# IntelLabs/bayesian-torch

Measured on AMD Instinct MI355X. Metric: MC-samples/sec (Bayesian-ResNet18, 224^2, bs=64), higher is better.
Workload: dtype bf16

## Files before the change

bayesian_torch_amd/_lib.py:

```python
import ctypes
import os

_HERE = os.path.dirname(os.path.abspath(__file__))
_LIB = None

KIND_REPARAM, KIND_FLIPOUT = 0, 1
ACT_F32, ACT_BF16 = 0, 1
PREC_F32, PREC_BF16, PREC_BF16X3 = 0, 1, 2
PREC_CODE = {"f32": 0, "bf16": 1, "bf16x3": 2}
FLAG_TRANSPOSED, FLAG_KL_ACCUM, FLAG_ROWFUSE, FLAG_OUT_F32, FLAG_OUT_BF16, FLAG_GATHER, FLAG_SWAP_SIGNS, FLAG_CONCURRENT = 1, 2, 4, 8, 16, 32, 64, 128
FLAG_REVERSE = 256
E_UNSUPPORTED = -3
STREAM_EPS_W, STREAM_EPS_B, STREAM_SIGN_IN, STREAM_SIGN_OUT = 0, 1, 2, 3
ABI_VERSION = 9
FLAG_LANES_SHIFT = 16
FLAG_LANES_MASK = 0xff << FLAG_LANES_SHIFT
SAMPLE_SKIP_MU = 1


class BtxError(RuntimeError):
    pass


class Geom(ctypes.Structure):
# ... 76 lines not shown


class OptimItem(ctypes.Structure):
    _fields_ = [("p", ctypes.c_void_p), ("g", ctypes.c_void_p), ("state0", ctypes.c_void_p), ("state1", ctypes.c_void_p),
                ("n", ctypes.c_int64)]


class BucketItem(ctypes.Structure):
    _fields_ = [("src", ctypes.c_void_p), ("offset", ctypes.c_int64), ("n", ctypes.c_int64)]


class OptimHyper(ctypes.Structure):
    _fields_ = [(n, ctypes.c_float) for n in ("neg_lr", "wd", "decay_mul", "one_m_b1", "b2", "one_m_b2", "eps", "neg_step_size",
                                              "bc2s", "momentum", "one_m_damp")] + \
               [("flags", ctypes.c_uint32), ("reserved", ctypes.c_uint32 * 4)]


OPT_MAXIMIZE, OPT_NESTEROV, OPT_DECOUPLED, OPT_FIRST_STEP, OPT_COUPLED_WD = 1, 2, 4, 8, 16
OPTIM_CHUNK, OPTIM_MAX_ITEMS = 4096, 65536
Q8_BIAS_NONE, Q8_BIAS_MU, Q8_BIAS_SIGMA_EPS = 0, 1, 2

EXPORTS = ("btx_abi_version", "btx_strerror", "btx_kl_workspace_bytes", "btx_kl_gauss", "btx_kl_model_workspace_bytes",
           "btx_kl_gauss_model", "btx_kl_gauss_model_bwd", "btx_contract_wgrad",
           "btx_contract_workspace_bytes", "btx_contract_fwd", "btx_contract_fwd_ex", "btx_contract_fwd_lanes", "btx_contract_pool_shape", "btx_contract_plan_info", "btx_out_shape", "btx_fill_eps", "btx_fill_sign", "btx_rho_grad",
           "btx_mc_packed_floats", "btx_mc_accumulate", "btx_mc_accumulate_lanes", "btx_sampled_w_bytes", "btx_sample_weights", "btx_sampled_w_bytes_lanes", "btx_sample_weights_lanes", "btx_rowfuse_pack", "btx_maxpool2d_cl", "btx_avgpool_global_cl",
           "btx_bn_workspace_bytes", "btx_bn_train_fwd", "btx_bn_train_bwd", "btx_dgrad_weights",
           "btx_wgrad_workspace_bytes", "btx_contract_wgrad_ws", "btx_maxpool2d_cl_train", "btx_maxpool2d_cl_bwd",
           "btx_lstm_workspace_bytes", "btx_lstm_fwd", "btx_lstm_train_saved_bytes", "btx_lstm_train_workspace_bytes",
           "btx_lstm_fwd_train", "btx_lstm_bwd",
           "btx_calib_workspace_bytes", "btx_avu_fwd", "btx_avu_bwd", "btx_eau_fwd", "btx_eau_bwd",
           "btx_q8_weight_row_bytes", "btx_q8_quantize_act", "btx_q8_sample_weights", "btx_q8_contract",
           "btx_q8_add", "btx_q8_contract_res", "btx_q8_maxpool2d_cl", "btx_q8_avgpool2d_cl",
           "btx_q8_sample_delta", "btx_q8_contract_flipout",
           "btx_optim_sgd", "btx_optim_adam", "btx_optim_grad_norm_workspace_bytes", "btx_optim_grad_norm",
           "btx_mcloss_workspace_bytes", "btx_mc_ce_fwd", "btx_mc_ce_bwd", "btx_avu_mc_fwd", "btx_avu_mc_bwd",
           "btx_bias_grad_workspace_bytes", "btx_bias_grad",
           "btx_bucket_pack", "btx_bucket_unpack")


def lib_path():
    return os.environ.get("BTX_LIB") or os.path.join(_HERE, "libbtx.so")


def lib():
    global _LIB
    if _LIB is not None:
        return _LIB
# ... 16 lines not shown
    L.btx_kl_gauss_model.restype = i32
    L.btx_kl_gauss_model.argtypes = [ctypes.POINTER(KlItem), i32, vp, vp, sz, vp]
    L.btx_kl_gauss_model_bwd.restype = i32
    L.btx_kl_gauss_model_bwd.argtypes = [ctypes.POINTER(KlItem), i32, vp, vp]
    L.btx_contract_wgrad.restype = i32
    L.btx_contract_wgrad.argtypes = [i32, ctypes.POINTER(Geom), vp, vp, vp, vp, vp, vp, ctypes.POINTER(Rng),
                                     ctypes.POINTER(Noise), i32, u32, vp]
    L.btx_contract_wgrad_ws.restype = i32
    L.btx_contract_wgrad_ws.argtypes = [i32, ctypes.POINTER(Geom), vp, vp, vp, vp, vp, vp, ctypes.POINTER(Rng),
                                        ctypes.POINTER(Noise), i32, u32, vp, sz, vp, vp, vp]
    L.btx_wgrad_workspace_bytes.restype = sz
    L.btx_wgrad_workspace_bytes.argtypes = [i32, ctypes.POINTER(Geom), i32, u32]
    L.btx_contract_workspace_bytes.restype = sz
    L.btx_contract_workspace_bytes.argtypes = [ctypes.POINTER(Geom), i32, i32, i32, u32]
    L.btx_contract_fwd.restype = i32
    L.btx_contract_fwd.argtypes = [i32, ctypes.POINTER(Geom), vp, vp, vp, vp, vp, vp, ctypes.POINTER(Rng),
                                   ctypes.POINTER(Noise), i32, i32, u32, vp, sz, vp]
    L.btx_contract_fwd_ex.restype = i32
    L.btx_contract_fwd_ex.argtypes = L.btx_contract_fwd.argtypes + [ctypes.POINTER(Epilogue)]
    L.btx_contract_fwd_lanes.restype = i32
    L.btx_contract_fwd_lanes.argtypes = L.btx_contract_fwd_ex.argtypes + [ctypes.POINTER(Lanes)]
    L.btx_contract_plan_info.restype = i32
    L.btx_contract_plan_info.argtypes = [i32, ctypes.POINTER(Geom), i32, i32, u32, ctypes.POINTER(Epilogue), ctypes.POINTER(PlanInfo)]
    L.btx_contract_pool_shape.restype = i32
    L.btx_contract_pool_shape.argtypes = [ctypes.POINTER(Geom), i32, i32, u32] + [ctypes.POINTER(ctypes.c_int32)] * 2
    L.btx_out_shape.restype = i32
    L.btx_out_shape.argtypes = [ctypes.POINTER(Geom), u32] + [ctypes.POINTER(ctypes.c_int32)] * 3
    L.btx_fill_eps.restype = i32
    L.btx_fill_eps.argtypes = [vp, sz, ctypes.POINTER(Rng), u32, vp]
    L.btx_rho_grad.restype = i32
    L.btx_rho_grad.argtypes = [vp, vp, vp, sz, ctypes.POINTER(Rng), u32, vp]
    L.btx_fill_sign.restype = i32
    L.btx_fill_sign.argtypes = [vp, sz, ctypes.POINTER(Rng), u32, vp]
    L.btx_mc_packed_floats.restype = sz
    L.btx_mc_packed_floats.argtypes = [i32, i32]
    L.btx_sampled_w_bytes.restype = sz
    L.btx_sampled_w_bytes.argtypes = [ctypes.POINTER(Geom), i32, i32]
    L.btx_sample_weights.restype = i32
    L.btx_sample_weights.argtypes = [ctypes.POINTER(SampleItem), i32, ctypes.POINTER(Rng), i32, vp]
    L.btx_sampled_w_bytes_lanes.restype = sz
    L.btx_sampled_w_bytes_lanes.argtypes = [ctypes.POINTER(Geom), i32, i32, i32]
    L.btx_sample_weights_lanes.restype = i32
    L.btx_sample_weights_lanes.argtypes = [ctypes.POINTER(SampleItem), i32, ctypes.POINTER(Rng), i32, vp, i32, u32]
    L.btx_rowfuse_pack.restype = i32
    L.btx_rowfuse_pack.argtypes = [vp, i32, ctypes.POINTER(ctypes.c_int64), i32, i32, i32, i32, vp, i32, i32, i32, i32, i32,
                                   i32, vp]
# ... 106 lines not shown
```

bayesian_torch_amd/csrc/btx_api.hip:

```cpp
#include <hip/hip_runtime.h>
#include <math.h>
#include <string.h>
#include "../../include/btx.h"
#include <stdlib.h>
#include "btx_contract.h"
#include "btx_rng.h"
#include "btx_presample.h"

using namespace btx;

static int contract_fwd_impl(int kind, const BtxGeom* g, const void* x, const float* mu_w, const float* rho_w,
                             const float* mu_b, const float* rho_b, void* out, const BtxRng* rng, const BtxNoise* noise,
                             int act_dtype, int prec, uint32_t flags, void* ws, size_t ws_bytes, void* stream,
                             const BtxEpilogue* ep, const BtxLanes* ln) {
  if (!g || !x || !mu_w || !rho_w || !out || !rng) return BTX_E_NULL;
  const int lanes = ln ? ln->n : 1;
  if ((mu_b == nullptr) != (rho_b == nullptr)) return BTX_E_NULL;
  const uintptr_t al = (uintptr_t)x | (uintptr_t)mu_w | (uintptr_t)rho_w | (uintptr_t)out |
                       (uintptr_t)(noise && noise->eps_w ? noise->eps_w : nullptr) |
                       (uintptr_t)(ep && ep->residual ? ep->residual : nullptr);
  FwdSel sel;
  int rc = select_fwd(kind, g, act_dtype, prec, flags, (al & 15) != 0, noise, ep, &sel);
  if (rc) return rc;
  const Plan& pl = sel.pl;
// ... 85 lines not shown
    case BTX_FAMILY_STEM: {
      const StemPlan& stp = sel.stp;
      p.pt_R = stp.R; p.pt_Rp = stp.Rp; p.pt_rtiles = stp.rtiles; p.pt_nw = stp.nw; p.pt_astage = stp.astage;
      p.st_sbytes = stp.sbytes; p.pt_lds = stp.lds; p.pt_PP = stp.patch_bytes;
      p.fd_rtiles = make_fastdiv((uint32_t)stp.rtiles);
      rc = launch(launch_contract_stem_f32, launch_contract_stem_bf16, launch_contract_stem_x3);
      break;
    }
    case BTX_FAMILY_PATCH:
    case BTX_FAMILY_TAPS:
    case BTX_FAMILY_TAPS2: {
      const PatchPlan& pt = sel.pt;
      p.pt_G = pt.G; p.pt_R = pt.R; p.pt_Rp = pt.Rp; p.pt_Wp = pt.Wp; p.pt_PP = pt.PP; p.pt_NI = pt.NI;
      p.fd_ptWp = make_fastdiv((uint32_t)pt.Wp); p.fd_ptRp = make_fastdiv((uint32_t)pt.Rp); p.fd_ptR = make_fastdiv((uint32_t)pt.R);
      p.fd_rtiles = make_fastdiv((uint32_t)pt.rtiles);
      p.pt_rtiles = pt.rtiles; p.pt_nw = pt.nw; p.pt_astage = pt.astage; p.pt_lds = pt.lds;
      p.pt_taps = pt.taps; p.pt_kg = pt.kg; p.pt_lds_g = pt.lds_g;
      p.pt_wide = (pt.taps == 33 || pt.taps == 332) ? pt.wide : 0;
      if (p.pt_wide) {
        p.fd_ntiles = make_fastdiv((uint32_t)(pl.ntiles / 2));
        p.fd_inner = make_fastdiv((uint32_t)((pl.ntiles / 2) * g->groups * pl.ksplits));
      }
      p.pt_tall = pt.tall; p.pt_P = pt.P; p.pt_Wt = pt.Wt; p.pt_ncs = pt.ncs;
      p.fd_P = make_fastdiv((uint32_t)pt.P); p.fd_Wt = make_fastdiv((uint32_t)pt.Wt); p.fd_ncs = make_fastdiv((uint32_t)pt.ncs);
      rc = launch(launch_contract_patch_f32, launch_contract_patch_bf16, launch_contract_patch_x3);
      break;
    }
    case BTX_FAMILY_GEMM8:
      p.pt_rtiles = sel.g8_pairs;
      p.fd_rtiles = make_fastdiv((uint32_t)sel.g8_pairs); p.fd_inner = make_fastdiv((uint32_t)(sel.g8_pairs * g->groups));
      rc = launch(launch_contract_gemm8_f32, launch_contract_gemm8_bf16, launch_contract_gemm8_x3);
      break;
    case BTX_FAMILY_DMA:
      rc = launch(launch_contract_dma_f32, launch_contract_dma_bf16, launch_contract_dma_x3);
      break;
    default: {
      const bool gen2 = sel.family == BTX_FAMILY_GATHER || (noise && (noise->eps_w || noise->sign_in));
      rc = (prec == BTX_PREC_BF16) ? launch_contract_bf16(kind, act_dtype == BTX_ACT_BF16, gen2, p, pl.nwg * lanes, st)
                                   : launch_contract_f32(kind, act_dtype == BTX_ACT_BF16, gen2, p, pl.nwg * lanes, st);
    }
  }
  if (rc) return rc;
  if (pl.ksplits > 1) {
    const long long total = (long long)pl.M * g->N;
    long long blocks = (total / 4 + 255) / 256;
    if (blocks > 2048) blocks = 2048;
// ... 122 lines not shown
```

bayesian_torch_amd/csrc/btx_contract.h:

```cpp
#pragma once
#include <hip/hip_runtime.h>
#include <stdint.h>
#include "btx_rng.h"
#include "btx_plan.h"

typedef __attribute__((ext_vector_type(8))) __bf16 bf16x8;
typedef __attribute__((ext_vector_type(4))) __bf16 bf16x4;
typedef __attribute__((ext_vector_type(4))) float f32x4;
typedef __attribute__((ext_vector_type(8))) float f32x8;
typedef __attribute__((ext_vector_type(16))) float f32x16;
typedef __attribute__((ext_vector_type(4))) uint32_t u32x4;
typedef __attribute__((ext_vector_type(2))) uint32_t u32x2;

namespace btx {

constexpr int NTHREADS = 512;
constexpr int ACTS_OFF = 0;
constexpr int SIGN_OFF = NG * BM * 16;
constexpr int WMU_OFF = SIGN_OFF + NG * BM * 4;
constexpr int WDL_OFF = WMU_OFF + NG * BN * 16;
constexpr int STAGE_BYTES = WDL_OFF + NG * BN * 16;
constexpr int LDS_BYTES = 2 * STAGE_BYTES;

struct FastDiv {
// ... 51 lines not shown
  int ep_relu;
  int out_bf16;
  int sign_unaligned;
  uint32_t x_bytes, w_bytes;
  int pt_G, pt_R, pt_Rp, pt_Wp, pt_PP, pt_NI, pt_rtiles;
  FastDiv fd_Wo, fd_Ho, fd_Do, fd_ptWp, fd_ptRp, fd_ptR;
  FastDiv fd_inner, fd_ksplits, fd_ntiles, fd_Cg, fd_KW, fd_KH, fd_rtiles;
  FastDiv fd_mtiles;
  int swap_signs;
  int par_major, par_Mq, par_Mqp, par_Hh, par_Wh;
  FastDiv fd_par_Mqp, fd_par_Hh, fd_par_Wh;
  FastDiv fd_sd, fd_sh, fd_sw;
  int wg_order;
  int pt_nw, pt_astage, pt_lds;
  int pt_kg;
  int pt_lds_g;
  int pt_taps;
  int pt_wide;
  int sp_Hq, sp_Wq;
  int st_sbytes;
  void* wt;
  uint32_t wt_bytes, wt_delta_off;
  int wt_ready;
  int pt_tall, pt_P, pt_Wt, pt_ncs;
  FastDiv fd_P, fd_Wt, fd_ncs;
  int lanes, lane_nwg;
  FastDiv fd_lane_nwg;
  long long lane_x, lane_out, lane_res, lane_wt, lane_partial;
  int lane_wt_delta;
  int reverse;
};

__device__ __forceinline__ uint32_t sample_word_scalar(const uint32_t* ptr) {
  return *(const __attribute__((address_space(4))) uint32_t*)(uintptr_t)ptr;
}

__device__ __forceinline__ int xcd_logical() {
  const int nwg = gridDim.x, L = blockIdx.x;
  const int q = nwg >> 3, r = nwg & 7, xcd = L & 7, slot = L >> 3;
  return (xcd < r ? xcd * (q + 1) : r * (q + 1) + (xcd - r) * q) + slot;
}

__device__ __forceinline__ ContractParams lane_view(const ContractParams& q, int& logical) {
  ContractParams p = q;
  if (q.reverse) logical = (int)gridDim.x - 1 - logical;
  if (q.lanes > 1) {
    uint32_t lane, loc;
// ... 687 lines not shown
```

bayesian_torch_amd/csrc/btx_contract_taps.h:

```cpp
#pragma once
#include <type_traits>
#include "btx_contract.h"
#include "btx_contract_dma.h"
#include "btx_epilogue.h"
#include "btx_mma.h"

namespace btx {

__device__ __forceinline__ void dma16s(__amdgpu_buffer_rsrc_t rsrc, uint32_t voff, uint32_t soff,
                                       unsigned char* lds_wave_base) {
  __builtin_amdgcn_raw_ptr_buffer_load_lds(rsrc, (__attribute__((address_space(3))) void*)lds_wave_base, 16, voff, soff,
                                           0, 0);
}

template <int N>
__device__ __forceinline__ void end_stage() {
  asm volatile("s_waitcnt vmcnt(%0)\n\ts_waitcnt lgkmcnt(0)\n\ts_barrier" ::"n"(N) : "memory");
}

template <int I, int N, class F>
__device__ __forceinline__ void static_for(F&& f) {
  if constexpr (I < N) {
    f(std::integral_constant<int, I>{});
    static_for<I + 1, N>(f);
// ... 30 lines not shown
  constexpr int ESZ = (int)sizeof(ACT);
  extern __shared__ __attribute__((aligned(16))) unsigned char smem_all[];

  uint32_t smp = p.sample;
  if (p.sample_ptr) smp = sample_word_scalar(p.sample_ptr);

  const int tid = threadIdx.x & 255;
  const int lane = tid & 63;
  const int l31 = lane & 31;
  const int h = lane >> 5;
  const int wave_all = __builtin_amdgcn_readfirstlane((int)(threadIdx.x >> 6));
  const int wave = wave_all & 3;
  const int kg = (KG == 1) ? 0 : (wave_all >> 2);
  unsigned char* const smem = smem_all + kg * p.pt_lds_g;

  uint32_t u_mtile, u_rem, u_split, u_ntile, u_group, u_t;
  const uint32_t ntg = (uint32_t)(WIDE ? p.ntiles >> 1 : p.ntiles);
  if (p.wg_order) fdivmod((uint32_t)logical, p.fd_mtiles, (uint32_t)p.mtiles, u_rem, u_mtile);
  else fdivmod((uint32_t)logical, p.fd_inner, ntg * (uint32_t)(p.groups * p.ksplits), u_mtile, u_rem);
  fdivmod(u_rem, p.fd_ksplits, (uint32_t)p.ksplits, u_t, u_split);
  fdivmod(u_t, p.fd_ntiles, ntg, u_group, u_ntile);
  const int mtile = (int)u_mtile, split = (int)u_split, ntile = (int)u_ntile, group = (int)u_group;

  const bool tall = p.pt_tall != 0;
  uint32_t u_ig, u_rt;
  if (tall) fdivmod((uint32_t)mtile, p.fd_ncs, (uint32_t)p.pt_ncs, u_rt, u_ig);
  else fdivmod((uint32_t)mtile, p.fd_rtiles, (uint32_t)p.pt_rtiles, u_ig, u_rt);
  const int img0 = tall ? 0 : (int)u_ig * p.pt_G, row0 = (int)u_rt * p.pt_R, col0 = tall ? (int)u_ig * p.pt_Wt : 0;
  auto patch_src = [&](int q, bool& ok) __attribute__((always_inline)) -> uint32_t {
    uint32_t ut, upc, ugi, upr;
    fdivmod((uint32_t)q, p.fd_ptWp, (uint32_t)p.pt_Wp, ut, upc);
    int img, ih, iw;
    if (tall) {
      fdivmod((uint32_t)row0 + ut, p.fd_P, (uint32_t)p.pt_P, ugi, upr);
      img = (int)ugi; ih = (int)upr - p.ph; iw = col0 + (int)upc - p.pw;
      ok = (int)ut < p.pt_Rp;
    } else {
      fdivmod(ut, p.fd_ptRp, (uint32_t)p.pt_Rp, ugi, upr);
      img = img0 + (int)ugi; ih = row0 + (int)upr - p.ph; iw = (int)upc - p.pw;
      ok = true;
    }
    ok = ok && img < p.NB && (unsigned)ih < (unsigned)p.H && (unsigned)iw < (unsigned)p.W;
    return (uint32_t)((img * p.H + ih) * p.W + iw);
  };
  const int ncb_total = p.Cg / BK;
  const int cb_per = p.kper / BK;
  const int cb0 = split * cb_per + kg * (cb_per / KG);
  const int ncb = (KG == 1) ? min(ncb_total, cb0 + cb_per) - cb0 : cb_per / KG;
  const int a_stage = p.pt_astage, s_stage = p.pt_astage >> 4;
  const int PT_A_OFF = 0, PT_S_OFF = 2 * a_stage, PT_W_OFF = 2 * a_stage + 2 * s_stage;
  const int PT_X_OFF = PT_W_OFF + PT_WD * DW_STAGE;

  const __amdgpu_buffer_rsrc_t x_rsrc = __builtin_amdgcn_make_buffer_rsrc((void*)p.x, 0, p.x_bytes, 0x00020000);
  const __amdgpu_buffer_rsrc_t wt_rsrc = __builtin_amdgcn_make_buffer_rsrc((void*)p.wt, 0, p.wt_bytes, 0x00020000);

  const uint32_t w_voff = (uint32_t)lane * 16u + (uint32_t)wave * 1024u;
  const uint32_t w_sbase = (uint32_t)(group * p.ntiles + (WIDE ? 2 * ntile : ntile)) * (uint32_t)(p.K / G) * 1024u;
// ... 69 lines not shown

  auto write_signs = [&](int slot, int cb) __attribute__((always_inline)) {
    if constexpr (KIND == 1) {
      unsigned char* ss = smem + PT_S_OFF + slot * s_stage;
#pragma unroll
      for (int j = 0; j < 2; ++j) {
        if (sg_ok[j]) {
          const uint32_t off = sg_off[j] + (uint32_t)(cb * BK);
          uint32_t w;
          if (p.sign_in) w = sign_word_explicit(p.sign_in, off, p.x_bytes / (uint32_t)ESZ);
          else w = btx_sign_word(off >> 5, rl.kin_a, rl.kin_b);
          if constexpr (G == 4) w <<= 8 * ((off >> 4) & 1);
          *(uint32_t*)(ss + (tid + NT * j) * 4) = w;
        }
      }
    }
  };

  int q0[MI];
#pragma unroll
  for (int mi = 0; mi < MI; ++mi) {
    const int pl = wave * 64 + mi * 32 + l31;
    uint32_t ut, uc, ugi, ur;
    if (tall) {
      fdivmod((uint32_t)pl, p.fd_Wt, (uint32_t)p.pt_Wt, ur, uc);
      q0[mi] = ((int)ur < p.pt_R) ? (int)ur * p.pt_Wp + (int)uc : 0;
    } else {
      fdivmod((uint32_t)pl, p.fd_Wo, (uint32_t)p.Wo, ut, uc);
      fdivmod(ut, p.fd_ptR, (uint32_t)p.pt_R, ugi, ur);
      const int c = (int)uc, r = (int)ur, gi = (int)ugi;
      const bool ok = (gi < p.pt_G) && (img0 + gi < p.NB) && (row0 + r < p.Ho);
      q0[mi] = ok ? (gi * p.pt_Rp + r) * p.pt_Wp + c : 0;
    }
  }
  const int row_step = p.dh * p.pt_Wp;

  constexpr bool ZI = (PREC == 1 && KG == 1);
  f32x16 accm[MI][2], accd[MI][2];
  auto clear_acc = [&](int a0) __attribute__((always_inline)) {
#pragma unroll
    for (int a = 0; a < MI; ++a)
#pragma unroll
      for (int b = 0; b < 2; ++b)
#pragma unroll
        for (int r = 0; r < 16; ++r)
          if (a >= a0) { accm[a][b][r] = 0.f; accd[a][b][r] = 0.f; }
  };
// ... 6 lines not shown
    const unsigned char* ss = smem + PT_S_OFF + aslot * s_stage;
    const unsigned char* ws = smem + PT_W_OFF + wsl * DW_STAGE;
    int q[MI];
#pragma unroll
    for (int mi = 0; mi < MI; ++mi) q[mi] = q0[mi] + toffv;
#pragma unroll
    for (int kk = 0; kk < NG / 2; ++kk) {
      const int row = 2 * kk + h;
#pragma unroll
      for (int mi = 0; mi < MIA; ++mi) f.a[kk][mi] = *(const u32x4*)(as + q[mi] * 64 + ((row ^ ((q[mi] >> 2) & 3)) * 16));
#pragma unroll
      for (int ni = 0; ni < 2; ++ni) f.wm[kk][ni] = *(const u32x4*)(ws + (row * BN + ni * 32 + l31) * 16);
    }
    if constexpr (KIND == 1) {
#pragma unroll
      for (int mi = 0; mi < MIA; ++mi) f.sw[mi] = *(const uint32_t*)(ss + q[mi] * 4);
    }
  };

  if (ncb > 0) {
    write_signs(0, cb0);
    asm volatile("s_waitcnt vmcnt(%0)\n\ts_waitcnt lgkmcnt(0)\n\ts_barrier" ::"n"(KG == 1 ? WOPS : 2 * WOPS) : "memory");
    Frag fa, fb;
    const int nvalid_px = tall ? p.pt_R * p.pt_Wt : min(p.pt_G, p.NB - img0) * min(p.pt_R, p.Ho - row0) * p.Wo;
    const bool mi1_dead = wave * 64 + 32 >= nvalid_px;
    auto kloop = [&](auto mia_tag) __attribute__((always_inline)) {
    constexpr int MIA = decltype(mia_tag)::value;
    if constexpr (KG == 1) load_frag(fa, 0, 0, 0, mia_tag);
    auto block = [&](auto par_tag, auto first_tag, int cbi, bool last) __attribute__((always_inline)) {
      constexpr int PAR = decltype(par_tag)::value;
      constexpr bool FIRST = decltype(first_tag)::value;
      static_for<0, T>([&](auto t_tag) __attribute__((always_inline)) {
        constexpr int t = decltype(t_tag)::value;
        constexpr int sp = (PAR * T + t) & 1;
        Frag& cur = (KG == 1 && sp) ? fb : fa;
        Frag& nxt = (KG == 1 && sp) ? fa : fb;
        asm volatile("" : "+v"(q0[0]), "+v"(q0[1]));
        constexpr int t3 = (t + 3) % T, c3 = (t + 3) / T;
        if constexpr (c3 == 0) {
          issue_w((uint32_t)t3, (uint32_t)(cb0 + cbi), (wslot + 3) & 3);
        } else {
          if (!last) issue_w((uint32_t)t3, (uint32_t)(cb0 + cbi + 1), (wslot + 3) & 3);
        }
        constexpr int KP = tp_pieces<T>(t);
        if constexpr (t < PST) {
          if (!last) {
            const uint32_t cboff = (uint32_t)((cb0 + cbi + 1) * BK * ESZ);
// ... 43 lines not shown
      block(P0{}, std::true_type{}, 0, ncb == 1);
      int cbi = 1;
      for (; cbi + 2 <= ncb; cbi += 2) {
        block(P1{}, std::false_type{}, cbi, false);
        block(P0{}, std::false_type{}, cbi + 1, cbi + 2 == ncb);
      }
      if (cbi < ncb) block(P1{}, std::false_type{}, cbi, true);
    } else {
      int cbi = 0;
      for (; cbi + 2 <= ncb; cbi += 2) {
        block(P0{}, std::false_type{}, cbi, false);
        block(P1{}, std::false_type{}, cbi + 1, cbi + 2 == ncb);
      }
      if (cbi < ncb) block(P0{}, std::false_type{}, cbi, true);
    }
    if (KG == 2 && kg == 0) asm volatile("s_barrier" ::: "memory");
    };
    if (mi1_dead) kloop(std::integral_constant<int, 1>{});
    else kloop(std::integral_constant<int, 2>{});
  }

  {
    BTX_SECTION_PARAMS(pe, logical2);
    const int nimg = min(pe.pt_G, pe.NB - img0), nrow = min(pe.pt_R, pe.Ho - row0);
    const int nvalid = nimg * nrow * pe.Wo;
    const uint32_t m0 = (uint32_t)(img0 * pe.Ho + row0) * (uint32_t)pe.Wo;
    const PixTall pmt = {pe, row0, col0};
    if constexpr (KG == 1) {
      if constexpr (WIDE) {
        float* const ba0 = (float*)(smem + NW * PT_EP_WAVE);
        float* const ba1 = ba0 + 4 * BN;
        {
          const bool has_bias = (split == 0) && (pe.mu_b != nullptr);
          const bool has_aff = (pe.ksplits == 1) && ((pe.ep_scale != nullptr) || (pe.ep_shift != nullptr));
          if (has_bias || has_aff) {
            if (tid < 64) ep_fill_constants<0>(pe, rl, ba0, tid, 2 * ntile, group, has_bias, has_aff);
            else if (tid < 128) ep_fill_constants<0>(pe, rl, ba1, tid - 64, 2 * ntile + 1, group, has_bias, has_aff);
          }
          __syncthreads();
        }
        if (tall) {
          staged_epilogue_pm<0, NW, PixTall>(pe, rl, accm, accm, smem, tid, wave, lane, 2 * ntile, group, split, pmt, -1, true, ba0);
          staged_epilogue_pm<0, NW, PixTall>(pe, rl, accd, accd, smem, tid, wave, lane, 2 * ntile + 1, group, split, pmt, -1, true, ba1);
        } else {
          staged_epilogue<0, NW>(pe, rl, accm, accm, smem, tid, wave, lane, 2 * ntile, group, split, m0, nvalid, -1, true, ba0);
          staged_epilogue<0, NW>(pe, rl, accd, accd, smem, tid, wave, lane, 2 * ntile + 1, group, split, m0, nvalid, -1, true, ba1);
        }
// ... 57 lines not shown
```

bayesian_torch_amd/csrc/btx_plan.cpp:

```cpp
#include <string.h>
#include "btx_plan.h"

namespace btx {

static inline long long plan_lanes(uint32_t flags) {
  const long long n = (flags >> BTX_FLAG_LANES_SHIFT) & 0xffu;
  return n > 1 ? n : 1;
}

static inline bool throughput_plan(uint32_t flags) { return (flags & BTX_FLAG_CONCURRENT) || plan_lanes(flags) > 1; }

static int split_k(long long base1, int units, int unit_cost, int max_split, bool full_splits, bool throughput, bool short_exit) {
  int ks = 1;
  long long best = -1;
  for (int c = 1; c <= max_split; ++c) {
    if (full_splits && units % c) continue;
    const int per = (units + c - 1) / c;
    const long long rounds = (base1 * c + SLOTS - 1) / SLOTS;
    const long long cost = rounds * (per * unit_cost + 4) + (c > 1 ? 1 : 0);
    if (best < 0 || cost < best) { best = cost; ks = c; }
    if (throughput && (base1 * c >= 64 || (short_exit && base1 * c >= 16 && per <= 16))) { ks = c; break; }
  }
  return ks;
}
// ... 40 lines not shown
static double tall_tile(const BtxGeom* g, const Plan& pl, int tp, int ppcap, PatchPlan* pt) {
  const int halo_r = (g->KH - 1) * g->dh, halo_c = (g->KW - 1) * g->dw;
  if (g->ph > halo_r) return 0.0;
  const int P = (g->H + g->ph > pl.Ho) ? g->H + g->ph : pl.Ho;
  const long long rows_total = (long long)(g->NB - 1) * P + pl.Ho;
  double best = 0.0;
  for (int ncs = 1; ncs <= 8; ++ncs) {
    const int Wt = (pl.Wo + ncs - 1) / ncs;
    if (Wt > tp || Wt < 4 || (ncs > 1 && Wt < 8)) continue;
    int R = tp / Wt;
    if (R > rows_total) R = (int)rows_total;
    while (R >= 1 && (R + halo_r) * (Wt + halo_c) > ppcap) --R;
    if (R < 1) continue;
    const long long rtiles = (rows_total + R - 1) / R;
    const double eff = (double)pl.M / ((double)rtiles * ncs * tp);
    if (eff > best * 1.01) {
      best = eff;
      pt->tall = 1; pt->P = P; pt->Wt = Wt; pt->ncs = ncs;
      pt->G = 1; pt->R = R; pt->Rp = R + halo_r; pt->Wp = Wt + halo_c; pt->PP = pt->Rp * pt->Wp;
      pt->rtiles = (int)rtiles;
    }
  }
  return best;
}
static bool patch_tile(const BtxGeom* g, const Plan& pl, int tp, int ppcap, PatchPlan* pt) {
  const int Ho = pl.Ho, Wo = pl.Wo;
  const int Wp = Wo + (g->KW - 1) * g->dw, halo_r = (g->KH - 1) * g->dh;
  if (Wo > tp || Wp * (1 + halo_r) > ppcap) return false;
  int G = 1, R;
  if (Ho * Wo <= tp / 2 || (Ho * Wo <= tp && (Ho + halo_r) * Wp <= ppcap)) {
    R = Ho;
    const int Rp = R + halo_r;
    if (Rp * Wp > ppcap) return false;
    G = tp / (Ho * Wo);
    if (G > ppcap / (Rp * Wp)) G = ppcap / (Rp * Wp);
    if (G > g->NB) G = g->NB;
    if (G < 1) return false;
  } else {
    int rmax = tp / Wo;
    const int rfit = ppcap / Wp - halo_r;
    if (rfit < rmax) rmax = rfit;
    if (rmax > Ho) rmax = Ho;
    if (rmax < 1) return false;
    const int nrt = (Ho + rmax - 1) / rmax;
    R = (Ho + nrt - 1) / nrt;
    auto mfma_tiles = [&](int r) {
// ... 44 lines not shown
}
static bool patch_split_k(const BtxGeom* g, int prec, uint32_t flags, int T, Plan* pl, const PatchPlan& pt) {
  const int bk = NG * (prec == BTX_PREC_BF16 ? 8 : 4);
  const int units = pl->Cg / bk / pt.kg;
  const long long base1 = patch_base1(g, *pl, pt);
  const long long base1n = throughput_plan(flags) ? (long long)pl->mtiles * pl->ntiles * g->groups : base1;
  int max_ks = 1;
  while (max_ks < units && max_ks < 32 && (units + max_ks) / (max_ks + 1) * T >= 4) ++max_ks;
  const int ks = split_k(base1n, units, T, max_ks, pt.kg == 2, throughput_plan(flags), false);
  const int per = (units + ks - 1) / ks;
  pl->kper = per * pt.kg * bk;
  pl->ksplits = (units + per - 1) / per;
  const long long nwg = base1 * pl->ksplits;
  if (nwg > 0x7fffffffLL) return false;
  pl->nwg = (int)nwg;
  return true;
}

static bool make_patch_plan(const BtxGeom* g, int act_dtype, int prec, uint32_t flags, Plan* pl, PatchPlan* pt, int kind = -1) {
  if (!patch_base_ok(g, act_dtype, prec, flags, pl, pt) || g->sh != 1 || g->sw != 1) return false;
  const int T = g->KH * g->KW;
  if (T < 2 || T > 64) return false;
  pt->tall = 0; pt->P = 1; pt->Wt = 1; pt->ncs = 1;
  if (patch_tile(g, *pl, 256, 352, pt)) pt->nw = 4;
  else if (patch_tile(g, *pl, 512, 960, pt)) pt->nw = 8;
  else return false;
  if (pt->nw == 4 && g->KH == 3 && g->KW == 3) {
    const long long mt_old = (long long)((g->NB + pt->G - 1) / pt->G) * pt->rtiles;
    const double eff_old = (double)pl->M / ((double)mt_old * 256.0);
    PatchPlan tp = *pt;
    const double eff_tall = tall_tile(g, *pl, 256, 352, &tp);
    if (eff_tall > eff_old * TALL_MIN_GAIN) *pt = tp;
  }
  if (!patch_lds(pt, 2, PT_WD, PT_MAXNI)) return false;
  pl->mtiles = pt->tall ? pt->rtiles * pt->ncs : ((g->NB + pt->G - 1) / pt->G) * pt->rtiles;
  pt->taps = (pt->nw == 4 && pt->NI <= 6 && g->KH == 3 && g->KW == 3) ? 33 : 0;
  if (pt->taps == 33) wide_tile(g, kind, act_dtype, prec, flags, *pl, pt);
  const int ncb = pl->Cg / (NG * (prec == BTX_PREC_BF16 ? 8 : 4));
  pt->kg = (pt->taps && !throughput_plan(flags) && patch_base1(g, *pl, *pt) * plan_lanes(flags) <= 256 && ncb >= 2 && (ncb % 2) == 0 &&
            2 * pt->lds_g <= 163840) ? 2 : 1;
  if (!patch_split_k(g, prec, flags, T, pl, *pt)) return false;
  if (pt->kg == 2) pt->lds = 2 * pt->lds_g;
  return true;
}

static bool make_patch2_plan(const BtxGeom* g, int act_dtype, int prec, uint32_t flags, Plan* pl, PatchPlan* pt, int kind = -1) {
  if (!patch_base_ok(g, act_dtype, prec, flags, pl, pt)) return false;
  if (g->KH != 3 || g->KW != 3 || g->sh != 2 || g->sw != 2 || g->ph != 1 || g->pw != 1 || g->dh != 1 || g->dw != 1) return false;
  BtxGeom gp = *g;
  gp.KH = 2; gp.KW = 2;
  if (!patch_tile(&gp, *pl, 256, 272, pt)) return false;
  pt->nw = 4;
  pt->tall = 0; pt->P = 1; pt->Wt = 1; pt->ncs = 1;
  if (!patch_lds(pt, 3, 3, 5)) return false;
  pl->mtiles = ((g->NB + pt->G - 1) / pt->G) * pt->rtiles;
  wide_tile(g, kind, act_dtype, prec, flags, *pl, pt);
  pt->taps = 332;
  pt->kg = 1;
  return patch_split_k(g, prec, flags, 9, pl, *pt);
}

static bool make_stem_plan(const BtxGeom* g, int act_dtype, int prec, const Plan& pl, StemPlan* st) {
  if (g->D != 1 || g->KD != 1 || pl.Do != 1 || g->groups != 1) return false;
  const int esz = (act_dtype == BTX_ACT_BF16) ? 2 : 4;
// ... 266 lines not shown
}

int btx_contract_plan_info(int kind, const BtxGeom* g, int act_dtype, int prec, uint32_t flags, const BtxEpilogue* ep,
                           BtxPlanInfo* out) {
  if (!g || !out) return BTX_E_NULL;
  memset(out, 0, sizeof(*out));
  FwdSel s;
  const int rc = select_fwd(kind, g, act_dtype, prec, flags, false, nullptr, ep, &s);
  if (rc) return rc;
  out->family = s.family;
  out->ksplits = s.pl.ksplits;
  out->kper = s.pl.kper;
  out->kgroups = s.pt.kg;
  out->wide = s.pt.wide;
  out->tall = s.pt.tall;
  out->par_major = s.par_major;
  out->pool_band = s.spp.PB;
  out->nwg = s.pl.nwg;
  out->lanes = (int32_t)plan_lanes(flags);
  out->ws_bytes = (uint64_t)s.need;
  return 0;
}

size_t btx_sampled_w_bytes(const BtxGeom* g, int kind, int prec) { return btx_sampled_w_bytes_lanes(g, kind, prec, 1); }

size_t btx_sampled_w_bytes_lanes(const BtxGeom* g, int kind, int prec, int lanes) {
  Plan pl;
  if (!g || lanes < 1 || lanes > 255 || make_plan(g, prec, 0, DBM, &pl)) return 0;
  size_t one = 0;
  const size_t tiles = patch_wt_bytes(pl, g, kind, prec, &one, lanes);
  return tiles + (kind == BTX_KIND_FLIPOUT ? one * (prec == BTX_PREC_BF16 ? 2 : 1) : 0);
}

}
```

bayesian_torch_amd/csrc/btx_plan.h:

```cpp
#pragma once
#include <stddef.h>
#include <stdint.h>
#include "../../include/btx.h"

namespace btx {

constexpr int BM = 256;
constexpr int BN = 64;
constexpr int NG = 4;
constexpr int DBM = 512;

constexpr int PT_WD = 4;
constexpr int PT_EP_ROW = 272;
constexpr int PT_EP_WAVE = 64 * PT_EP_ROW;
constexpr int PT_MAXNI = 8;

constexpr long long SLOTS = 256;
constexpr double TALL_MIN_GAIN = 1.15;
constexpr int GEMM8_MIN_K = 128;
constexpr double WG_MAJOR_MIB = 3.0;

struct Plan {
  int Do, Ho, Wo, Cg, Ng, M, K, mtiles, ntiles, ksplits, kper, nwg;
};

struct PatchPlan {
  int G, R, Rp, Wp, PP, NI, rtiles, nw, astage, lds;
  int taps, kg, lds_g;
  int wide;
  int tall, P, Wt, ncs;
};

struct StemPlan {
  int R, Rp, rtiles, nw, astage, sbytes, lds, patch_bytes, nwg;
};

struct StemPoolPlan {
  int PB, bands, Rp, astage, sbytes, lds, patch_bytes, nwg, Hq, Wq;
};

struct FwdSel {
  int family;
  Plan pl;
  int par_major;
  int par_mqp, g8_pairs, out_bf16;
  StemPlan stp;
  StemPoolPlan spp;
  PatchPlan pt;
  size_t need, wt_off, wt_one, wt_all;
};
static inline bool uses_tiles(int family) { return family >= BTX_FAMILY_DMA; }

int select_fwd(int kind, const BtxGeom* g, int act_dtype, int prec, uint32_t flags, bool unaligned, const BtxNoise* noise,
               const BtxEpilogue* ep, FwdSel* s);

// ... 6 lines not shown
```

include/btx.h:

```cpp
#ifndef BTX_H_
#define BTX_H_

#include <stddef.h>
#include <stdint.h>

#ifdef __cplusplus
extern "C" {
#endif

#define BTX_ABI_VERSION 9

#define BTX_E_NULL        (-1)
#define BTX_E_SHAPE       (-2)
#define BTX_E_UNSUPPORTED (-3)
#define BTX_E_WORKSPACE   (-4)
#define BTX_E_DTYPE       (-5)
#define BTX_E_ALIGN       (-6)

#define BTX_KIND_REPARAM 0
#define BTX_KIND_FLIPOUT 1
#define BTX_ACT_F32  0
#define BTX_ACT_BF16 1
#define BTX_PREC_F32  0
#define BTX_PREC_BF16 1
// ... 109 lines not shown
#define BTX_FAMILY_REGSTAGE  1
#define BTX_FAMILY_DMA       2
#define BTX_FAMILY_GEMM8     3
#define BTX_FAMILY_PATCH     4
#define BTX_FAMILY_TAPS      5
#define BTX_FAMILY_TAPS2     6
#define BTX_FAMILY_STEM      7
#define BTX_FAMILY_STEM_POOL 8
typedef struct BtxPlanInfo {
  int32_t  family;
  int32_t  ksplits;
  int32_t  kper;
  int32_t  kgroups;
  int32_t  wide;
  int32_t  tall;
  int32_t  par_major;
  int32_t  pool_band;
  int32_t  nwg;
  int32_t  lanes;
  uint64_t ws_bytes;
} BtxPlanInfo;
int btx_contract_plan_info(int kind, const BtxGeom* g, int act_dtype, int prec, uint32_t flags,
                           const BtxEpilogue* ep , BtxPlanInfo* out);

int btx_contract_wgrad(int kind, const BtxGeom* g, const void* x, const void* dy, float* dw_mu, float* dw_delta,
                       float* db_mu, float* db_delta, const BtxRng* rng, const BtxNoise* noise ,
                       int act_dtype, uint32_t flags, void* stream);
size_t btx_wgrad_workspace_bytes(int kind, const BtxGeom* g, int act_dtype, uint32_t flags);
int btx_contract_wgrad_ws(int kind, const BtxGeom* g, const void* x, const void* dy, float* dw_mu, float* dw_delta,
                          float* db_mu, float* db_delta, const BtxRng* rng, const BtxNoise* noise ,
                          int act_dtype, uint32_t flags, void* ws, size_t ws_bytes, const float* rho_w ,
                          float* drho , void* stream);

typedef struct BtxSampleItem {
  const BtxGeom* geom;
  const float*   mu_w;
  const float*   rho_w;
  void*          out;
  int32_t        kind;
  uint32_t       layer_id;
  int32_t        src_KW, src_C;
} BtxSampleItem;
size_t btx_sampled_w_bytes(const BtxGeom* g, int kind, int prec);
int btx_sample_weights(const BtxSampleItem* items_host, int n_items, const BtxRng* rng ,
                       int prec, void* stream);
#define BTX_SAMPLE_SKIP_MU 1u
// ... 193 lines not shown
```

Measured before the change: 1930.

## Add flat cross-image row tiling for taps conv kernel

Adds a 'flat' patch tiling mode (tall==2) that treats all NB*Ho output rows as one sequence, so a tile may span image boundaries and small late-layer feature maps fill the 256-pixel MFMA tile better. The planner picks flat tiling only when its modeled MFMA-tile count and workgroup count are no worse than the incumbent plan, and recomputes nwg. The kernel gains extra index arithmetic for virtual-row mapping and padded cross-image halos, which may add LDS traffic. A host debug export for tile mapping is also added.

```diff
diff --git a/bayesian_torch_amd/_lib.py b/bayesian_torch_amd/_lib.py
--- a/bayesian_torch_amd/_lib.py
+++ b/bayesian_torch_amd/_lib.py
@@ -122,7 +122,7 @@
 
 EXPORTS = ("btx_abi_version", "btx_strerror", "btx_kl_workspace_bytes", "btx_kl_gauss", "btx_kl_model_workspace_bytes",
            "btx_kl_gauss_model", "btx_kl_gauss_model_bwd", "btx_contract_wgrad",
-           "btx_contract_workspace_bytes", "btx_contract_fwd", "btx_contract_fwd_ex", "btx_contract_fwd_lanes", "btx_contract_pool_shape", "btx_contract_plan_info", "btx_out_shape", "btx_fill_eps", "btx_fill_sign", "btx_rho_grad",
+           "btx_contract_workspace_bytes", "btx_contract_fwd", "btx_contract_fwd_ex", "btx_contract_fwd_lanes", "btx_contract_pool_shape", "btx_contract_plan_info", "btx_flat_tile_map", "btx_out_shape", "btx_fill_eps", "btx_fill_sign", "btx_rho_grad",
            "btx_mc_packed_floats", "btx_mc_accumulate", "btx_mc_accumulate_lanes", "btx_sampled_w_bytes", "btx_sample_weights", "btx_sampled_w_bytes_lanes", "btx_sample_weights_lanes", "btx_rowfuse_pack", "btx_maxpool2d_cl", "btx_avgpool_global_cl",
            "btx_bn_workspace_bytes", "btx_bn_train_fwd", "btx_bn_train_bwd", "btx_dgrad_weights",
            "btx_wgrad_workspace_bytes", "btx_contract_wgrad_ws", "btx_maxpool2d_cl_train", "btx_maxpool2d_cl_bwd",
@@ -185,6 +185,8 @@
     L.btx_contract_fwd_lanes.argtypes = L.btx_contract_fwd_ex.argtypes + [ctypes.POINTER(Lanes)]
     L.btx_contract_plan_info.restype = i32
     L.btx_contract_plan_info.argtypes = [i32, ctypes.POINTER(Geom), i32, i32, u32, ctypes.POINTER(Epilogue), ctypes.POINTER(PlanInfo)]
+    L.btx_flat_tile_map.restype = i32
+    L.btx_flat_tile_map.argtypes = [i32, ctypes.POINTER(Geom), i32, i32, u32, i32] + [ctypes.POINTER(ctypes.c_int32)] * 3
     L.btx_contract_pool_shape.restype = i32
     L.btx_contract_pool_shape.argtypes = [ctypes.POINTER(Geom), i32, i32, u32] + [ctypes.POINTER(ctypes.c_int32)] * 2
     L.btx_out_shape.restype = i32
diff --git a/bayesian_torch_amd/csrc/btx_api.hip b/bayesian_torch_amd/csrc/btx_api.hip
--- a/bayesian_torch_amd/csrc/btx_api.hip
+++ b/bayesian_torch_amd/csrc/btx_api.hip
@@ -131,6 +131,7 @@
         p.fd_inner = make_fastdiv((uint32_t)((pl.ntiles / 2) * g->groups * pl.ksplits));
       }
       p.pt_tall = pt.tall; p.pt_P = pt.P; p.pt_Wt = pt.Wt; p.pt_ncs = pt.ncs;
+      p.pt_rows = pt.tall == 2 ? g->NB * pl.Ho : pl.Ho;
       p.fd_P = make_fastdiv((uint32_t)pt.P); p.fd_Wt = make_fastdiv((uint32_t)pt.Wt); p.fd_ncs = make_fastdiv((uint32_t)pt.ncs);
       rc = launch(launch_contract_patch_f32, launch_contract_patch_bf16, launch_contract_patch_x3);
       break;
diff --git a/bayesian_torch_amd/csrc/btx_contract.h b/bayesian_torch_amd/csrc/btx_contract.h
--- a/bayesian_torch_amd/csrc/btx_contract.h
+++ b/bayesian_torch_amd/csrc/btx_contract.h
@@ -97,7 +97,7 @@
   void* wt;
   uint32_t wt_bytes, wt_delta_off;
   int wt_ready;
-  int pt_tall, pt_P, pt_Wt, pt_ncs;
+  int pt_tall, pt_P, pt_Wt, pt_ncs, pt_rows;
   FastDiv fd_P, fd_Wt, fd_ncs;
   int lanes, lane_nwg;
   FastDiv fd_lane_nwg;
diff --git a/bayesian_torch_amd/csrc/btx_contract_taps.h b/bayesian_torch_amd/csrc/btx_contract_taps.h
--- a/bayesian_torch_amd/csrc/btx_contract_taps.h
+++ b/bayesian_torch_amd/csrc/btx_contract_taps.h
@@ -76,17 +76,25 @@
   fdivmod(u_t, p.fd_ntiles, ntg, u_group, u_ntile);
   const int mtile = (int)u_mtile, split = (int)u_split, ntile = (int)u_ntile, group = (int)u_group;
 
-  const bool tall = p.pt_tall != 0;
+  const bool tall = p.pt_tall == 1, flat = p.pt_tall == 2, vpatch = p.pt_tall != 0;
   uint32_t u_ig, u_rt;
-  if (tall) fdivmod((uint32_t)mtile, p.fd_ncs, (uint32_t)p.pt_ncs, u_rt, u_ig);
+  if (vpatch) fdivmod((uint32_t)mtile, p.fd_ncs, (uint32_t)p.pt_ncs, u_rt, u_ig);
   else fdivmod((uint32_t)mtile, p.fd_rtiles, (uint32_t)p.pt_rtiles, u_ig, u_rt);
-  const int img0 = tall ? 0 : (int)u_ig * p.pt_G, row0 = (int)u_rt * p.pt_R, col0 = tall ? (int)u_ig * p.pt_Wt : 0;
+  const int img0 = vpatch ? 0 : (int)u_ig * p.pt_G, row0 = (int)u_rt * p.pt_R, col0 = vpatch ? (int)u_ig * p.pt_Wt : 0;
+  struct FlatDivDev {
+    const ContractParams& p;
+    __device__ __forceinline__ void by_Ho(uint32_t x, uint32_t& q, uint32_t& r) const { fdivmod(x, p.fd_Ho, (uint32_t)p.Ho, q, r); }
+    __device__ __forceinline__ void by_Wo(uint32_t x, uint32_t& q, uint32_t& r) const { fdivmod(x, p.fd_Wo, (uint32_t)p.Wo, q, r); }
+  };
+  const FlatDivDev fdm = {p};
+  const FlatMap fmap = {p.Ho, p.Wo, p.pt_P, p.pt_Wp, p.pt_R, p.NB * p.Ho};
+  const int vrow0 = flat ? flat_vrow(fmap, row0, fdm) : row0;
   auto patch_src = [&](int q, bool& ok) __attribute__((always_inline)) -> uint32_t {
     uint32_t ut, upc, ugi, upr;
     fdivmod((uint32_t)q, p.fd_ptWp, (uint32_t)p.pt_Wp, ut, upc);
     int img, ih, iw;
-    if (tall) {
-      fdivmod((uint32_t)row0 + ut, p.fd_P, (uint32_t)p.pt_P, ugi, upr);
+    if (vpatch) {
+      fdivmod((uint32_t)vrow0 + ut, p.fd_P, (uint32_t)p.pt_P, ugi, upr);
       img = (int)ugi; ih = (int)upr - p.ph; iw = col0 + (int)upc - p.pw;
       ok = (int)ut < p.pt_Rp;
     } else {
@@ -202,7 +210,9 @@
   for (int mi = 0; mi < MI; ++mi) {
     const int pl = wave * 64 + mi * 32 + l31;
     uint32_t ut, uc, ugi, ur;
-    if (tall) {
+    if (flat) {
+      q0[mi] = flat_slot(fmap, row0, vrow0, pl, fdm);
+    } else if (tall) {
       fdivmod((uint32_t)pl, p.fd_Wt, (uint32_t)p.pt_Wt, ur, uc);
       q0[mi] = ((int)ur < p.pt_R) ? (int)ur * p.pt_Wp + (int)uc : 0;
     } else {
@@ -255,7 +265,7 @@
     write_signs(0, cb0);
     asm volatile("s_waitcnt vmcnt(%0)\n\ts_waitcnt lgkmcnt(0)\n\ts_barrier" ::"n"(KG == 1 ? WOPS : 2 * WOPS) : "memory");
     Frag fa, fb;
-    const int nvalid_px = tall ? p.pt_R * p.pt_Wt : min(p.pt_G, p.NB - img0) * min(p.pt_R, p.Ho - row0) * p.Wo;
+    const int nvalid_px = tall ? p.pt_R * p.pt_Wt : min(p.pt_G, p.NB - img0) * min(p.pt_R, p.pt_rows - row0) * p.Wo;
     const bool mi1_dead = wave * 64 + 32 >= nvalid_px;
     auto kloop = [&](auto mia_tag) __attribute__((always_inline)) {
     constexpr int MIA = decltype(mia_tag)::value;
@@ -345,7 +355,7 @@
 
   {
     BTX_SECTION_PARAMS(pe, logical2);
-    const int nimg = min(pe.pt_G, pe.NB - img0), nrow = min(pe.pt_R, pe.Ho - row0);
+    const int nimg = min(pe.pt_G, pe.NB - img0), nrow = min(pe.pt_R, pe.pt_rows - row0);
     const int nvalid = nimg * nrow * pe.Wo;
     const uint32_t m0 = (uint32_t)(img0 * pe.Ho + row0) * (uint32_t)pe.Wo;
     const PixTall pmt = {pe, row0, col0};
diff --git a/bayesian_torch_amd/csrc/btx_plan.cpp b/bayesian_torch_amd/csrc/btx_plan.cpp
--- a/bayesian_torch_amd/csrc/btx_plan.cpp
+++ b/bayesian_torch_amd/csrc/btx_plan.cpp
@@ -86,6 +86,46 @@
     }
   }
   return best;
+}
+static long long wg_mfma_tiles(long long n) {
+  long long t = 0;
+  for (int w = 0; w < 4; ++w) t += (w * 64 + 32 < n) ? 2 : 1;
+  return t;
+}
+static void tile_plan_cost(const BtxGeom* g, const Plan& pl, const PatchPlan& pt, long long* mfma, long long* wgs) {
+  long long m = 0, w = 0;
+  if (pt.tall == 1) {
+    w = (long long)pt.rtiles * pt.ncs;
+    m = w * wg_mfma_tiles((long long)pt.R * pt.Wt);
+  } else if (pt.tall == 2) {
+    const long long rows = (long long)g->NB * pl.Ho;
+    for (long long r0 = 0; r0 < rows; r0 += pt.R, ++w) m += wg_mfma_tiles((rows - r0 < pt.R ? rows - r0 : pt.R) * pl.Wo);
+  } else {
+    for (int i0 = 0; i0 < g->NB; i0 += pt.G)
+      for (int r0 = 0; r0 < pl.Ho; r0 += pt.R, ++w)
+        m += wg_mfma_tiles((long long)(g->NB - i0 < pt.G ? g->NB - i0 : pt.G) * (pl.Ho - r0 < pt.R ? pl.Ho - r0 : pt.R) * pl.Wo);
+  }
+  *mfma = m; *wgs = w;
+}
+static bool flat_tile(const BtxGeom* g, const Plan& pl, int tp, int ppcap, PatchPlan* pt) {
+  const int halo_r = (g->KH - 1) * g->dh, halo_c = (g->KW - 1) * g->dw;
+  if (g->ph > halo_r || pl.Wo > tp) return false;
+  const int P = (g->H + g->ph > pl.Ho) ? g->H + g->ph : pl.Ho;
+  const long long rows = (long long)g->NB * pl.Ho;
+  const int Wp = pl.Wo + halo_c;
+  int R = tp / pl.Wo, Rp = 0;
+  if (R > rows) R = (int)rows;
+  for (; R >= 1; --R) {
+    long long cross = (R + pl.Ho - 2) / pl.Ho;
+    if (cross > g->NB - 1) cross = g->NB - 1;
+    const long long rp = R + cross * (P - pl.Ho) + halo_r;
+    if (rp * Wp <= ppcap) { Rp = (int)rp; break; }
+  }
+  if (R < 1) return false;
+  pt->tall = 2; pt->P = P; pt->Wt = pl.Wo; pt->ncs = 1;
+  pt->G = 1; pt->R = R; pt->Rp = Rp; pt->Wp = Wp; pt->PP = Rp * Wp;
+  pt->rtiles = (int)((rows + R - 1) / R);
+  return true;
 }
 static bool patch_tile(const BtxGeom* g, const Plan& pl, int tp, int ppcap, PatchPlan* pt) {
   const int Ho = pl.Ho, Wo = pl.Wo;
@@ -176,6 +216,7 @@
   const int T = g->KH * g->KW;
   if (T < 2 || T > 64) return false;
   pt->tall = 0; pt->P = 1; pt->Wt = 1; pt->ncs = 1;
+  int mt_order = 0;
   if (patch_tile(g, *pl, 256, 352, pt)) pt->nw = 4;
   else if (patch_tile(g, *pl, 512, 960, pt)) pt->nw = 8;
   else return false;
@@ -185,15 +226,30 @@
     PatchPlan tp = *pt;
     const double eff_tall = tall_tile(g, *pl, 256, 352, &tp);
     if (eff_tall > eff_old * TALL_MIN_GAIN) *pt = tp;
+    PatchPlan fp = *pt;
+    if (flat_tile(g, *pl, 256, 352, &fp)) {
+      long long m_inc, w_inc, m_flat, w_flat;
+      tile_plan_cost(g, *pl, *pt, &m_inc, &w_inc);
+      tile_plan_cost(g, *pl, fp, &m_flat, &w_flat);
+      if (m_flat <= m_inc && w_flat <= w_inc) {
+        mt_order = (int)w_inc;
+        *pt = fp;
+      }
+    }
   }
   if (!patch_lds(pt, 2, PT_WD, PT_MAXNI)) return false;
-  pl->mtiles = pt->tall ? pt->rtiles * pt->ncs : ((g->NB + pt->G - 1) / pt->G) * pt->rtiles;
+  const int mt_launch = pt->tall ? pt->rtiles * pt->ncs : ((g->NB + pt->G - 1) / pt->G) * pt->rtiles;
+  pl->mtiles = mt_order ? mt_order : mt_launch;
   pt->taps = (pt->nw == 4 && pt->NI <= 6 && g->KH == 3 && g->KW == 3) ? 33 : 0;
   if (pt->taps == 33) wide_tile(g, kind, act_dtype, prec, flags, *pl, pt);
   const int ncb = pl->Cg / (NG * (prec == BTX_PREC_BF16 ? 8 : 4));
   pt->kg = (pt->taps && !throughput_plan(flags) && patch_base1(g, *pl, *pt) * plan_lanes(flags) <= 256 && ncb >= 2 && (ncb % 2) == 0 &&
             2 * pt->lds_g <= 163840) ? 2 : 1;
   if (!patch_split_k(g, prec, flags, T, pl, *pt)) return false;
+  if (mt_order) {
+    pl->mtiles = mt_launch;
+    pl->nwg = (int)(patch_base1(g, *pl, *pt) * pl->ksplits);
+  }
   if (pt->kg == 2) pt->lds = 2 * pt->lds_g;
   return true;
 }
@@ -506,6 +562,27 @@
   return 0;
 }
 
+int btx_flat_tile_map(int kind, const BtxGeom* g, int act_dtype, int prec, uint32_t flags, int32_t tile, int32_t info[8],
+                      int32_t q0[256], int32_t pix[256]) {
+  if (!g || !info) return BTX_E_NULL;
+  FwdSel s;
+  const int rc = select_fwd(kind, g, act_dtype, prec, flags, false, nullptr, nullptr, &s);
+  if (rc) return rc;
+  if (s.family != BTX_FAMILY_TAPS || s.pt.tall != 2) return BTX_E_UNSUPPORTED;
+  const PatchPlan& pt = s.pt;
+  if (tile < 0 || tile >= pt.rtiles) return BTX_E_SHAPE;
+  const FlatMap f = {s.pl.Ho, s.pl.Wo, pt.P, pt.Wp, pt.R, g->NB * s.pl.Ho};
+  const FlatDivHost dm = {s.pl.Ho, s.pl.Wo};
+  const int row0 = tile * pt.R, vrow0 = flat_vrow(f, row0, dm), nvalid = flat_nvalid(f, row0);
+  info[0] = pt.R; info[1] = pt.Rp; info[2] = pt.Wp; info[3] = pt.PP; info[4] = pt.P; info[5] = pt.rtiles;
+  info[6] = nvalid; info[7] = vrow0;
+  for (int pl = 0; pl < 256; ++pl) {
+    if (q0) q0[pl] = flat_slot(f, row0, vrow0, pl, dm);
+    if (pix) pix[pl] = pl < nvalid ? row0 * s.pl.Wo + pl : -1;
+  }
+  return 0;
+}
+
 size_t btx_sampled_w_bytes(const BtxGeom* g, int kind, int prec) { return btx_sampled_w_bytes_lanes(g, kind, prec, 1); }
 
 size_t btx_sampled_w_bytes_lanes(const BtxGeom* g, int kind, int prec, int lanes) {
diff --git a/bayesian_torch_amd/csrc/btx_plan.h b/bayesian_torch_amd/csrc/btx_plan.h
--- a/bayesian_torch_amd/csrc/btx_plan.h
+++ b/bayesian_torch_amd/csrc/btx_plan.h
@@ -31,6 +31,38 @@
   int tall, P, Wt, ncs;
 };
 
+#if defined(__HIPCC__)
+#define BTX_PLAN_HD __host__ __device__
+#else
+#define BTX_PLAN_HD
+#endif
+struct FlatMap {
+  int Ho, Wo, P, Wp, R, rows;
+};
+struct FlatDivHost {
+  int Ho, Wo;
+  void by_Ho(uint32_t x, uint32_t& q, uint32_t& r) const { q = x / (uint32_t)Ho; r = x % (uint32_t)Ho; }
+  void by_Wo(uint32_t x, uint32_t& q, uint32_t& r) const { q = x / (uint32_t)Wo; r = x % (uint32_t)Wo; }
+};
+template <class DM>
+BTX_PLAN_HD inline int flat_vrow(const FlatMap& f, int r, const DM& dm) {
+  uint32_t img, oh;
+  dm.by_Ho((uint32_t)r, img, oh);
+  return (int)img * f.P + (int)oh;
+}
+BTX_PLAN_HD inline int flat_nvalid(const FlatMap& f, int row0) {
+  const int n = f.rows - row0;
+  return (n < f.R ? n : f.R) * f.Wo;
+}
+template <class DM>
+BTX_PLAN_HD inline int flat_slot(const FlatMap& f, int row0, int vrow0, int pl, const DM& dm) {
+  uint32_t r, c;
+  dm.by_Wo((uint32_t)pl, r, c);
+  const int rr = row0 + (int)r;
+  if ((int)r >= f.R || rr >= f.rows) return 0;
+  return (flat_vrow(f, rr, dm) - vrow0) * f.Wp + (int)c;
+}
+
 struct StemPlan {
   int R, Rp, rtiles, nw, astage, sbytes, lds, patch_bytes, nwg;
 };
diff --git a/include/btx.h b/include/btx.h
--- a/include/btx.h
+++ b/include/btx.h
@@ -155,6 +155,8 @@
 } BtxPlanInfo;
 int btx_contract_plan_info(int kind, const BtxGeom* g, int act_dtype, int prec, uint32_t flags,
                            const BtxEpilogue* ep , BtxPlanInfo* out);
+int btx_flat_tile_map(int kind, const BtxGeom* g, int act_dtype, int prec, uint32_t flags, int32_t tile, int32_t info[8],
+                      int32_t q0[256], int32_t pix[256]);
 
 int btx_contract_wgrad(int kind, const BtxGeom* g, const void* x, const void* dy, float* dw_mu, float* dw_delta,
                        float* db_mu, float* db_delta, const BtxRng* rng, const BtxNoise* noise ,
```

Result: faster. 1984 (median of 6 runs) (+2.8%).
